# mhalushka/miRge3.0

Hardware: NVIDIA B200
Metric: M reads/s trim+collapse+annotate (higher is better)
Workload: dtype u8/int32

## Files before the change

### mirge3.0_b200/csrc/annotate.cu

```cuda
#include "common.cuh"

#include "annotate_verify.cuh"


__global__ void __launch_bounds__(256)
lib_kmers_kernel(mirge_library lib, uint32_t *__restrict__ kmer, uint8_t *__restrict__ valid) {
  const uint32_t p = blockIdx.x * 256u + threadIdx.x;
  if (p >= lib.n_bases) return;
  const uint32_t r = find_ref(lib, p);
  const uint32_t end = lib.d_ref_off[r + 1];
  uint32_t k = 0, v = 0;
  for (uint32_t i = 0; i < 16; ++i) {
    const uint32_t q = p + i;
    if (q >= end) break;
    if ((lib.d_nmask[q >> 5] >> (q & 31)) & 1u) break;
    k |= lib_base(lib.d_packed, q) << (2 * (15 - i));
    ++v;
  }
  kmer[p] = k;
  valid[p] = (uint8_t)v;
}

extern "C" int mirge_lib_kmers(mirge_ctx *ctx, const mirge_library *lib, uint32_t *d_kmer, uint8_t *d_valid, void *stream_) {
  if (!ctx) return MIRGE_ERR_ARG;
  if (!lib || !lib->d_packed || !lib->d_nmask || !lib->d_ref_off || !lib->d_ref_block || !d_kmer || !d_valid)
    MIRGE_FAIL(ctx, MIRGE_ERR_ARG, "lib_kmers: null buffer");
  if (lib->n_bases == 0 || lib->n_refs == 0) return MIRGE_OK;
  cudaStream_t stream = (cudaStream_t)stream_;
  MIRGE_CUDA(ctx, cudaSetDevice(ctx->device));
  lib_kmers_kernel<<<(lib->n_bases + 255) / 256, 256, 0, stream>>>(*lib, d_kmer, d_valid);
  MIRGE_LAUNCH_CHECK(ctx, "lib_kmers_kernel");
  return MIRGE_OK;
}

__global__ void __launch_bounds__(256)
lib_filter_kernel(const uint32_t *__restrict__ kmer, const uint8_t *__restrict__ valid, uint32_t n, uint32_t bases,
                  uint32_t *__restrict__ filter) {
  const uint32_t p = blockIdx.x * 256u + threadIdx.x;
  if (p >= n || valid[p] < bases) return;
  const uint32_t fi = bases >= 16 ? kmer[p] : (kmer[p] >> (32 - 2 * bases));
  atomicOr(filter + (fi >> 5), 1u << (fi & 31));
}

extern "C" int mirge_lib_filter(mirge_ctx *ctx, const uint32_t *d_kmer, const uint8_t *d_valid, uint32_t n_bases, uint32_t prefix_bases,
                                uint32_t *d_filter, void *stream_) {
  if (!ctx) return MIRGE_ERR_ARG;
  if (!d_kmer || !d_valid || !d_filter) MIRGE_FAIL(ctx, MIRGE_ERR_ARG, "lib_filter: null buffer");
  if (prefix_bases < 4 || prefix_bases > 16) MIRGE_FAIL(ctx, MIRGE_ERR_ARG, "lib_filter: prefix length must be 4..16");
  if (n_bases == 0) return MIRGE_OK;
  cudaStream_t stream = (cudaStream_t)stream_;
  MIRGE_CUDA(ctx, cudaSetDevice(ctx->device));
  MIRGE_CUDA(ctx, cudaMemsetAsync(d_filter, 0, (size_t)1 << (2 * prefix_bases - 3), stream));
  lib_filter_kernel<<<(n_bases + 255) / 256, 256, 0, stream>>>(d_kmer, d_valid, n_bases, prefix_bases, d_filter);
  MIRGE_LAUNCH_CHECK(ctx, "lib_filter_kernel");
  return MIRGE_OK;
}

__device__ __forceinline__ uint32_t mix32(uint32_t x) {
  x ^= x >> 16;
  x *= 0x7feb352du;
  x ^= x >> 15;
  x *= 0x846ca68bu;
  x ^= x >> 16;
  return x;
}
__device__ __forceinline__ bool filter16_pass(const mirge_library &lib, uint32_t kmer) {
  const uint32_t fi = mix32(kmer) >> (32 - lib.filter16_bits);
  return (lib.d_filter16[fi >> 5] >> (fi & 31)) & 1u;
}

__global__ void __launch_bounds__(256)
lib_filter16_kernel(const uint32_t *__restrict__ kmer, const uint8_t *__restrict__ valid, uint32_t n, uint32_t bits,
                    uint32_t *__restrict__ filter) {
  const uint32_t p = blockIdx.x * 256u + threadIdx.x;
  if (p >= n || valid[p] < 16) return;
  const uint32_t fi = mix32(kmer[p]) >> (32 - bits);
  atomicOr(filter + (fi >> 5), 1u << (fi & 31));
}

extern "C" int mirge_lib_filter16(mirge_ctx *ctx, const uint32_t *d_kmer, const uint8_t *d_valid, uint32_t n_bases, uint32_t bits,
                                  uint32_t *d_filter16, void *stream_) {
  if (!ctx) return MIRGE_ERR_ARG;
  if (!d_kmer || !d_valid || !d_filter16) MIRGE_FAIL(ctx, MIRGE_ERR_ARG, "lib_filter16: null buffer");
  if (bits < 16 || bits > 30) MIRGE_FAIL(ctx, MIRGE_ERR_ARG, "lib_filter16: 16..30 bits");
  cudaStream_t stream = (cudaStream_t)stream_;
  MIRGE_CUDA(ctx, cudaSetDevice(ctx->device));
  MIRGE_CUDA(ctx, cudaMemsetAsync(d_filter16, 0, (size_t)1 << (bits - 3), stream));
  if (n_bases == 0) return MIRGE_OK;
  lib_filter16_kernel<<<(n_bases + 255) / 256, 256, 0, stream>>>(d_kmer, d_valid, n_bases, bits, d_filter16);
  MIRGE_LAUNCH_CHECK(ctx, "lib_filter16_kernel");
  return MIRGE_OK;
}


#define MAX_PIECES 4
#define MAX_ROUNDS 10

struct RoundSet {
  int n;
  mirge_library lib[MAX_ROUNDS];
  mirge_round_policy pol[MAX_ROUNDS];
};

#define COOP_QW 6
struct WarpScratch {
  uint32_t qw[32][COOP_QW], qnx[32][COOP_QW];
  uint32_t lo[32][MAX_PIECES], hi[32][MAX_PIECES], off[32][MAX_PIECES];
  uint32_t len[32];
  uint32_t pref[33];
  unsigned long long best[32];
};

__device__ __forceinline__ uint64_t search_round(const mirge_library &lib, const mirge_round_policy &pol, bool active,
                                                 const uint32_t *qw, const uint32_t *qnx, int L, bool has_exc, WarpScratch &ws,
                                                 bool &republish, int lane) {
  uint32_t p_lo[MAX_PIECES], p_hi[MAX_PIECES], p_off[MAX_PIECES];
#pragma unroll
  for (int i = 0; i < MAX_PIECES; ++i) p_lo[i] = p_hi[i] = p_off[i] = 0;
  if (lib.max_ref_len && (uint32_t)L > lib.max_ref_len) active = false;
  const int R = pol.seed_len == 0 ? L : min(pol.seed_len, L);
  const int np = pol.seed_mm + 1;
  const bool degenerate = active && (R < MIN_SEED * np);
  const int nw = (L + 15) >> 4;
  if (active && !degenerate) {
    for (int pi = 0; pi < np; ++pi) {
      const int a = piece_bound(pi, R, np), b = piece_bound(pi + 1, R, np);
      const int s = min(16, b - a);
      if (has_exc && query_has_n(qnx, a, b)) continue;
      const uint32_t span = (s == 16) ? 0u : ((1u << (2 * (16 - s))) - 1u);
      const uint32_t k_lo = query_kmer16(qw, a, nw) & ~span, k_hi = k_lo | span;
      if (s == 16 && lib.filter16_bits && lib.filter_bases < 16) {
        if (!filter16_pass(lib, k_lo)) continue;
      } else if (lib.filter_bases && (uint32_t)s >= lib.filter_bases) {
        const uint32_t fi = lib.filter_bases >= 16 ? k_lo : (k_lo >> (32 - 2 * lib.filter_bases));
        if (!((lib.d_filter[fi >> 5] >> (fi & 31)) & 1u)) continue;
      }
      const uint32_t bsh = 32 - lib.bucket_bits;
      uint32_t l = lib.d_idx_bucket[k_lo >> bsh], h = lib.d_idx_bucket[(k_hi >> bsh) + 1];
      const uint32_t hi0 = h;
      while (l < h) { const uint32_t mid = (l + h) >> 1; if (lib.d_idx_kmer[mid] < k_lo) l = mid + 1; else h = mid; }
      p_lo[pi] = l;
      h = hi0;
      while (l < h) { const uint32_t mid = (l + h) >> 1; if (lib.d_idx_kmer[mid] <= k_hi) l = mid + 1; else h = mid; }
      p_hi[pi] = l;
      p_off[pi] = (uint32_t)a;
    }
  }
  uint64_t best = MIRGE_NO_HIT;
  uint32_t total = 0;
#pragma unroll
  for (int i = 0; i < MAX_PIECES; ++i) total += p_hi[i] - p_lo[i];
  const bool shared = active && !degenerate && total > 0 && nw <= COOP_QW;
  if (degenerate) {
    for (uint32_t r = 0; r < lib.n_refs; ++r) {
      const uint32_t lo = lib.d_ref_off[r], hi = lib.d_ref_off[r + 1];
      for (uint64_t a = lo; a + L <= hi; ++a) {
        const uint64_t h = verify(lib, qw, qnx, L, pol, R, a, (uint32_t)a);
        if (h < best) best = h;
      }
    }
  } else if (active && total > 0 && !shared) {
#pragma unroll
    for (int pi = 0; pi < MAX_PIECES; ++pi)
      for (uint32_t e = p_lo[pi]; e < p_hi[pi]; ++e) {
        const uint32_t pos = lib.d_idx_pos[e];
        if (pos < p_off[pi]) continue;
        const uint64_t h = verify(lib, qw, qnx, L, pol, R, pos - p_off[pi], pos);
        if (h < best) best = h;
      }
  }
  const unsigned sm = __ballot_sync(0xffffffffu, shared);
  if (sm == 0) return best;
  uint32_t incl = shared ? total : 0u;
#pragma unroll
  for (int d = 1; d < 32; d <<= 1) {
    const uint32_t x = __shfl_up_sync(0xffffffffu, incl, d);
    if (lane >= d) incl += x;
  }
  const uint32_t T = __shfl_sync(0xffffffffu, incl, 31);
  ws.pref[lane + 1] = incl;
  if (lane == 0) ws.pref[0] = 0;
  if (shared) {
    if (republish) {
      for (int w = 0; w < nw; ++w) { ws.qw[lane][w] = qw[w]; ws.qnx[lane][w] = qnx[w]; }
      republish = false;
    }
#pragma unroll
    for (int pi = 0; pi < MAX_PIECES; ++pi) { ws.lo[lane][pi] = p_lo[pi]; ws.hi[lane][pi] = p_hi[pi]; ws.off[lane][pi] = p_off[pi]; }
    ws.len[lane] = (uint32_t)L;
    ws.best[lane] = MIRGE_NO_HIT;
  }
  __syncwarp();
  for (uint32_t w = lane; w < T; w += 32) {
    int o = 0;
#pragma unroll
    for (int st = 16; st > 0; st >>= 1)
      if (ws.pref[o + st] <= w) o += st;
    uint32_t j = w - ws.pref[o];
    int pi = 0;
#pragma unroll
    for (int q = 0; q < MAX_PIECES - 1; ++q) {
      const uint32_t c = ws.hi[o][pi] - ws.lo[o][pi];
      if (j >= c && pi == q) { j -= c; ++pi; }
    }
    const uint32_t pos = lib.d_idx_pos[ws.lo[o][pi] + j], off = ws.off[o][pi];
    if (pos < off) continue;
    const int oL = (int)ws.len[o];
    const int oR = pol.seed_len == 0 ? oL : min(pol.seed_len, oL);
    const uint64_t h = verify(lib, ws.qw[o], ws.qnx[o], oL, pol, oR, pos - off, pos);
    if (h != MIRGE_NO_HIT) atomicMin(&ws.best[o], (unsigned long long)h);
  }
  __syncwarp();
  if (shared) {
    const uint64_t b = ws.best[lane];
    if (b < best) best = b;
  }
  return best;
}

__global__ void __launch_bounds__(ANN_THREADS, 10)
annotate_kernel(const __grid_constant__ RoundSet rs, mirge_table t, uint64_t n_keys, uint8_t *__restrict__ annot_round,
                uint64_t *__restrict__ hit) {
  __shared__ WarpScratch s_ws[ANN_THREADS / 32];
  const uint64_t slot = (uint64_t)blockIdx.x * ANN_THREADS + threadIdx.x;
  const int lane = threadIdx.x & 31, warp = threadIdx.x >> 5;
  const bool in_range = slot < n_keys;
  const uint64_t id = slot;
  uint32_t qw[QW_MAX], qnx[QW_MAX];
  KeyView kv;
  kv.pay = kv.exc = nullptr; kv.len = kv.nexc = 0;
  int cur_qs = -1, cur_qe = -1, tlen = -1;
  uint32_t state = 0xFF;
  if (in_range) {
    kv = key_view(t.d_arena + t.d_key_ref[id]);
    state = annot_round[id];
  }
  const int len = kv.len, nexc = kv.nexc;
  uint64_t my_hit = MIRGE_NO_HIT;
  int my_round = -1;
  bool republish = true;
  for (int ri = 0; ri < rs.n; ++ri) {
    const mirge_round_policy &pol = rs.pol[ri];
    bool active = in_range;
    if (active) {
      if (pol.select == MIRGE_SELECT_LEN_LT26) active = len < 26;
      else if (pol.select == MIRGE_SELECT_LEN_GT25) active = len > 25;
      else active = state == 0xFF;
    }
    int L = 0;
    if (active) {
      int qs, qe;
      active = round_window(kv, pol, tlen, qs, qe);
      if (active) {
        L = qe - qs;
        if (qs != cur_qs || qe != cur_qe) {
          build_query(kv, qs, qe, qw, qnx);
          cur_qs = qs;
          cur_qe = qe;
          republish = true;
        }
      }
    }
    const uint64_t best = search_round(rs.lib[ri], pol, active, qw, qnx, L, nexc > 0, s_ws[warp], republish, lane);
    if (active && best != MIRGE_NO_HIT) {
      state = (uint32_t)pol.round;
      my_round = pol.round;
      my_hit = best;
    }
  }
  if (my_round >= 0) {
    annot_round[id] = (uint8_t)my_round;
    hit[id] = my_hit;
  }
}

__global__ void __launch_bounds__(ANN_THREADS)
allhits_kernel(mirge_library lib, mirge_round_policy pol, mirge_table t, const uint32_t *__restrict__ ids, uint64_t n,
               const uint64_t *__restrict__ hit, int fill, uint32_t *__restrict__ counts, const uint64_t *__restrict__ offs,
               uint64_t *__restrict__ out) {
  const uint64_t i = (uint64_t)blockIdx.x * ANN_THREADS + threadIdx.x;
  if (i >= n) return;
  const uint32_t id = ids[i];
  const uint64_t want_mm = hit[id] >> 56;
  const KeyView kv = key_view(t.d_arena + t.d_key_ref[id]);
  uint32_t qw[QW_MAX], qnx[QW_MAX];
  int tlen = -1, qs, qe;
  uint32_t k = 0;
  const uint64_t o0 = fill ? offs[i] : 0;
  if (round_window(kv, pol, tlen, qs, qe)) {
    build_query(kv, qs, qe, qw, qnx);
    const int L = qe - qs, nw = (L + 15) >> 4;
    const int R = pol.seed_len == 0 ? L : min(pol.seed_len, L);
    const int np = pol.seed_mm + 1;
#define ALLHITS_TAKE(h_)                                    \
    if ((h_) != MIRGE_NO_HIT && ((h_) >> 56) == want_mm) {  \
      if (fill) out[o0 + k] = (h_);                         \
      ++k;                                                  \
    }
    if (R < MIN_SEED * np) {
      for (uint32_t r = 0; r < lib.n_refs; ++r) {
        const uint32_t lo = lib.d_ref_off[r], hi = lib.d_ref_off[r + 1];
        for (uint64_t a = lo; a + L <= hi; ++a) {
          const uint64_t h = verify(lib, qw, qnx, L, pol, R, a, (uint32_t)a);
          ALLHITS_TAKE(h)
        }
      }
    } else {
      for (int pi = 0; pi < np; ++pi) {
        const int a = piece_bound(pi, R, np), b = piece_bound(pi + 1, R, np);
        const int s = min(16, b - a);
        if (kv.nexc > 0 && query_has_n(qnx, a, b)) continue;
        const uint32_t span = (s == 16) ? 0u : ((1u << (2 * (16 - s))) - 1u);
        const uint32_t k_lo = query_kmer16(qw, a, nw) & ~span, k_hi = k_lo | span;
        const uint32_t bsh = 32 - lib.bucket_bits;
        uint32_t l = lib.d_idx_bucket[k_lo >> bsh], h = lib.d_idx_bucket[(k_hi >> bsh) + 1];
        const uint32_t hi0 = h;
        while (l < h) { const uint32_t mid = (l + h) >> 1; if (lib.d_idx_kmer[mid] < k_lo) l = mid + 1; else h = mid; }
        const uint32_t e0 = l;
        h = hi0;
        while (l < h) { const uint32_t mid = (l + h) >> 1; if (lib.d_idx_kmer[mid] <= k_hi) l = mid + 1; else h = mid; }
        for (uint32_t e = e0; e < l; ++e) {
          const uint32_t pos = lib.d_idx_pos[e];
          if (pos < (uint32_t)a) continue;
          const uint64_t hh = verify(lib, qw, qnx, L, pol, R, pos - (uint32_t)a, pos);
          ALLHITS_TAKE(hh)
        }
      }
    }
#undef ALLHITS_TAKE
  }
  if (!fill) counts[i] = k;
}


__device__ __forceinline__ uint32_t round_mask(const RoundSet &rs, const KeyView &kv, uint32_t state) {
  uint32_t qw[QW_MAX], qnx[QW_MAX];
  int cur_qs = -1, cur_qe = -1, tlen = -1;
  const int len = kv.len;
  const bool has_exc = kv.nexc > 0;
  uint32_t mask = 0;
  for (int ri = 0; ri < rs.n; ++ri) {
    const mirge_round_policy &pol = rs.pol[ri];
    const mirge_library &lib = rs.lib[ri];
    bool active;
    if (pol.select == MIRGE_SELECT_LEN_LT26) active = len < 26;
    else if (pol.select == MIRGE_SELECT_LEN_GT25) active = len > 25;
    else active = state == 0xFF;
    if (!active) continue;
    int qs, qe;
    if (!round_window(kv, pol, tlen, qs, qe)) continue;
    const int L = qe - qs;
    if (lib.max_ref_len && (uint32_t)L > lib.max_ref_len) continue;
    if (qs != cur_qs || qe != cur_qe) {
      build_query(kv, qs, qe, qw, qnx);
      cur_qs = qs;
      cur_qe = qe;
    }
    const int R = pol.seed_len == 0 ? L : min(pol.seed_len, L);
    const int np = pol.seed_mm + 1;
    const int nw = (L + 15) >> 4;
    bool pass = false;
    if (R < MIN_SEED * np) {
      pass = true;
    } else {
      for (int pi = 0; pi < np; ++pi) {
        const int a = piece_bound(pi, R, np), b = piece_bound(pi + 1, R, np);
        const int s = min(16, b - a);
        if (has_exc && query_has_n(qnx, a, b)) continue;
        if (s == 16 && lib.filter16_bits && lib.filter_bases < 16) {
          pass |= filter16_pass(lib, query_kmer16(qw, a, nw));
        } else if (lib.filter_bases && (uint32_t)s >= lib.filter_bases) {
          const uint32_t span = (s == 16) ? 0u : ((1u << (2 * (16 - s))) - 1u);
          const uint32_t k_lo = query_kmer16(qw, a, nw) & ~span;
          const uint32_t fi = lib.filter_bases >= 16 ? k_lo : (k_lo >> (32 - 2 * lib.filter_bases));
          pass |= ((lib.d_filter[fi >> 5] >> (fi & 31)) & 1u) != 0u;
        } else {
          pass = true;
        }
      }
    }
    if (pass) mask |= 1u << ri;
  }
  return mask;
}

#define LEAN_WORDS 8
#define MASK_THREADS 256
template <int S>
__device__ __forceinline__ uint32_t lean_word16(const uint32_t *col, int p) {
  const int wi = p >> 4, sh = 2 * (p & 15);
  return __funnelshift_r(col[wi * S], col[(wi + 1) * S], sh);
}
template <int S>
__device__ __forceinline__ uint32_t lean_kmer16(const uint32_t *col, int p) {
  const uint32_t v = lean_word16<S>(col, p);
  const uint32_t r = __brev(v);
  return ((r >> 1) & 0x55555555u) | ((r & 0x55555555u) << 1);
}

template <int S>
__device__ __forceinline__ bool lean_window(const uint32_t *col, int len, const mirge_round_policy &pol, int &tlen, int &qs, int &qe) {
  qs = 0;
  qe = len;
  if (pol.strip_polyT) {
    if (tlen < 0) {
      int tpos = len;
      while (tpos > 0 && ((col[((tpos - 1) >> 4) * S] >> (2 * ((tpos - 1) & 15))) & 3u) == 3u) --tpos;
      tlen = tpos;
    }
    if (len - tlen < 3) return false;
    qe = tlen;
  }
  qs += pol.trim5;
  qe -= pol.trim3;
  return qe > qs;
}

__device__ __forceinline__ uint32_t round_mask_lean(const RoundSet &rs, const uint32_t *col, int len, uint32_t state) {
  int tlen = -1;
  uint32_t mask = 0;
  for (int ri = 0; ri < rs.n; ++ri) {
    const mirge_round_policy &pol = rs.pol[ri];
    const mirge_library &lib = rs.lib[ri];
    bool active;
    if (pol.select == MIRGE_SELECT_LEN_LT26) active = len < 26;
    else if (pol.select == MIRGE_SELECT_LEN_GT25) active = len > 25;
    else active = state == 0xFF;
    if (!active) continue;
    int qs, qe;
    if (!lean_window<MASK_THREADS>(col, len, pol, tlen, qs, qe)) continue;
    const int L = qe - qs;
    if (lib.max_ref_len && (uint32_t)L > lib.max_ref_len) continue;
    const int R = pol.seed_len == 0 ? L : min(pol.seed_len, L);
    const int np = pol.seed_mm + 1;
    bool pass = false;
    if (R < MIN_SEED * np) {
      pass = true;
    } else {
      int a = 0;
      for (int pi = 0; pi < np; ++pi) {
        const int b = piece_bound(pi + 1, R, np);
        const int s = min(16, b - a);
        const uint32_t k16 = lean_kmer16<MASK_THREADS>(col, qs + a);
        if (s == 16 && lib.filter16_bits && lib.filter_bases < 16) {
          pass |= filter16_pass(lib, k16);
        } else if (lib.filter_bases && (uint32_t)s >= lib.filter_bases) {
          const uint32_t fi = lib.filter_bases >= 16 ? k16 : (k16 >> (32 - 2 * lib.filter_bases));
          pass |= ((lib.d_filter[fi >> 5] >> (fi & 31)) & 1u) != 0u;
        } else {
          pass = true;
        }
        a = b;
      }
    }
    if (pass) mask |= 1u << ri;
  }
  return mask;
}

__global__ void __launch_bounds__(MASK_THREADS)
annot_mask_kernel(const __grid_constant__ RoundSet rs, mirge_table t, uint64_t n_keys, const uint8_t *__restrict__ annot_round,
                  uint16_t *__restrict__ masks) {
  __shared__ uint32_t s_pay[LEAN_WORDS + 2][MASK_THREADS];
  const uint64_t id = (uint64_t)blockIdx.x * MASK_THREADS + threadIdx.x;
  if (id >= n_keys) return;
  const uint32_t *key = t.d_arena + t.d_key_ref[id];
  const uint32_t state = annot_round[id];
  const KeyView kv = key_view(key);
  const int npay = (kv.len + 15) >> 4;
  uint32_t mask;
  if (kv.nexc == 0 && npay <= LEAN_WORDS) {
    uint32_t *col = &s_pay[0][threadIdx.x];
#pragma unroll
    for (int w = 0; w < LEAN_WORDS + 2; ++w) col[w * MASK_THREADS] = w < npay ? kv.pay[w] : 0u;
    mask = round_mask_lean(rs, col, kv.len, state);
  } else {
    mask = round_mask(rs, kv, state);
  }
  masks[id] = (uint16_t)mask;
}

#ifndef LEAN_MAX_CAND
#define LEAN_MAX_CAND 12
#endif
template <int S>
__device__ __forceinline__ bool search_lean(const mirge_library &lib, const mirge_round_policy &pol, const uint32_t *col, int qs,
                                            int L, uint64_t &best) {
  if (lib.max_ref_len && (uint32_t)L > lib.max_ref_len) return true;
  const int R = pol.seed_len == 0 ? L : min(pol.seed_len, L);
  const int np = pol.seed_mm + 1;
  if (R < MIN_SEED * np) return false;
  uint32_t p_lo[MAX_PIECES], p_hi[MAX_PIECES];
  uint32_t total = 0;
  int a = 0;
#pragma unroll
  for (int pi = 0; pi < MAX_PIECES; ++pi) {
    p_lo[pi] = p_hi[pi] = 0;
    if (pi < np) {
      const int b = piece_bound(pi + 1, R, np);
      const int s = min(16, b - a);
      const uint32_t k16 = lean_kmer16<S>(col, qs + a);
      const uint32_t span = (s == 16) ? 0u : ((1u << (2 * (16 - s))) - 1u);
      const uint32_t k_lo = k16 & ~span, k_hi = k_lo | span;
      bool look = true;
      if (s == 16 && lib.filter16_bits && lib.filter_bases < 16) {
        look = filter16_pass(lib, k_lo);
      } else if (lib.filter_bases && (uint32_t)s >= lib.filter_bases) {
        const uint32_t fi = lib.filter_bases >= 16 ? k_lo : (k_lo >> (32 - 2 * lib.filter_bases));
        look = (lib.d_filter[fi >> 5] >> (fi & 31)) & 1u;
      }
      if (look) {
        const uint32_t bsh = 32 - lib.bucket_bits;
        uint32_t l = lib.d_idx_bucket[k_lo >> bsh], h = lib.d_idx_bucket[(k_hi >> bsh) + 1];
        const uint32_t hi0 = h;
        while (l < h) { const uint32_t mid = (l + h) >> 1; if (lib.d_idx_kmer[mid] < k_lo) l = mid + 1; else h = mid; }
        p_lo[pi] = l;
        h = hi0;
        while (l < h) { const uint32_t mid = (l + h) >> 1; if (lib.d_idx_kmer[mid] <= k_hi) l = mid + 1; else h = mid; }
        p_hi[pi] = l;
        total += p_hi[pi] - p_lo[pi];
      }
      a = b;
    }
  }
  if (total > LEAN_MAX_CAND) return false;
  const int nw = (L + 15) >> 4;
  a = 0;
#pragma unroll
  for (int pi = 0; pi < MAX_PIECES; ++pi) {
    if (pi < np) {
      for (uint32_t e = p_lo[pi]; e < p_hi[pi]; ++e) {
        const uint32_t pos = lib.d_idx_pos[e];
        if (pos < (uint32_t)a) continue;
        const uint64_t astart = pos - (uint32_t)a;
        int mm = 0, smm = 0;
        for (int w = 0; w < nw && mm >= 0; ++w) {
          uint32_t x = lean_word16<S>(col, qs + 16 * w) ^ lib_word16(lib.d_packed, astart + 16 * (uint64_t)w);
          x = (x | (x >> 1)) & 0x55555555u;
          const int rem = L - 16 * w;
          if (rem < 16) x &= (1u << (2 * rem)) - 1u;
          if (x) {
            mm += __popc(x);
            const int srem = R - 16 * w;
            if (srem >= 16) smm += __popc(x);
            else if (srem > 0) smm += __popc(x & ((1u << (2 * srem)) - 1u));
            if (mm > pol.total_mm || smm > pol.seed_mm) mm = -1;
          }
        }
        if (mm < 0) continue;
        const uint32_t r = find_ref(lib, pos);
        const uint32_t rlo = lib.d_ref_off[r], rhi = lib.d_ref_off[r + 1];
        if (astart < rlo || astart + (uint64_t)L > rhi) continue;
        if (ref_has_n(lib, astart, astart + L)) continue;
        const uint64_t hword = ((uint64_t)mm << 56) | ((uint64_t)r << 28) | (uint64_t)(astart - rlo);
        if (hword < best) best = hword;
      }
      a = piece_bound(pi + 1, R, np);
    }
  }
  return true;
}

#define SUB_KEYS 256
struct WarpTile {
  uint16_t mask[SUB_KEYS];
  uint16_t list[SUB_KEYS];
  uint8_t state[SUB_KEYS];
  uint32_t pay[LEAN_WORDS + 2][32];
};

struct GeneralList {
  unsigned long long *count;
  uint32_t *id;
  uint8_t *round;
};

__global__ void __launch_bounds__(ANN_THREADS, 10)
annot_search_kernel(const __grid_constant__ RoundSet rs, mirge_table t, uint64_t n_keys, const uint16_t *__restrict__ masks,
                    uint8_t *__restrict__ annot_round, uint64_t *__restrict__ hit, const GeneralList gl) {
  __shared__ WarpTile s_wt[ANN_THREADS / 32];
  const int lane = threadIdx.x & 31, warp = threadIdx.x >> 5;
  WarpTile &W = s_wt[warp];
  const uint64_t tile0 = ((uint64_t)blockIdx.x * (ANN_THREADS / 32) + warp) * SUB_KEYS;
  if (tile0 >= n_keys) return;
  const uint32_t n_tile = (uint32_t)min((uint64_t)SUB_KEYS, n_keys - tile0);
  uint32_t any = 0;
  for (uint32_t k = lane; k < SUB_KEYS; k += 32) {
    const uint32_t m = k < n_tile ? masks[tile0 + k] : 0u;
    W.mask[k] = (uint16_t)m;
    W.state[k] = k < n_tile ? annot_round[tile0 + k] : (uint8_t)0;
    any |= m;
  }
  any = __reduce_or_sync(0xffffffffu, any);
  __syncwarp();
  for (int ri = 0; ri < rs.n; ++ri) {
    if (!((any >> ri) & 1u)) continue;
    const mirge_round_policy &pol = rs.pol[ri];
    uint32_t cnt = 0;
    for (uint32_t k0 = 0; k0 < SUB_KEYS; k0 += 32) {
      const uint32_t k = k0 + lane;
      bool p = (W.mask[k] >> ri) & 1u;
      if (p && pol.select == MIRGE_SELECT_UNANNOTATED) p = W.state[k] == 0xFF;
      const unsigned bal = __ballot_sync(0xffffffffu, p);
      if (p) W.list[cnt + __popc(bal & ((1u << lane) - 1u))] = (uint16_t)k;
      cnt += __popc(bal);
    }
    __syncwarp();
    for (uint32_t base = 0; base < cnt; base += 32) {
      const uint32_t idx = base + lane;
      const bool active = idx < cnt;
      const uint32_t k = active ? W.list[idx] : 0u;
      const uint64_t id = tile0 + k;
      uint64_t best = MIRGE_NO_HIT;
      bool general = false;
      if (active) {
        const KeyView kv = key_view(t.d_arena + t.d_key_ref[id]);
        const int npay = (kv.len + 15) >> 4;
        general = true;
        if (kv.nexc == 0 && npay <= LEAN_WORDS) {
          uint32_t *col = &W.pay[0][lane];
#pragma unroll
          for (int w = 0; w < LEAN_WORDS + 2; ++w) col[w * 32] = w < npay ? kv.pay[w] : 0u;
          int qs, qe, tlen = -1;
          if (!lean_window<32>(col, kv.len, pol, tlen, qs, qe)) general = false;
          else general = !search_lean<32>(rs.lib[ri], pol, col, qs, qe - qs, best);
        }
      }
      const unsigned gm = __ballot_sync(0xffffffffu, general);
      if (gm) {
        const int leader = __ffs(gm) - 1;
        unsigned long long gb = 0;
        if (lane == leader) gb = atomicAdd(gl.count, (unsigned long long)__popc(gm));
        gb = __shfl_sync(0xffffffffu, gb, leader);
        if (general) {
          const unsigned long long e = gb + __popc(gm & ((1u << lane) - 1u));
          gl.id[e] = (uint32_t)id;
          gl.round[e] = (uint8_t)ri;
          W.mask[k] = 0;
        }
      }
      if (active && best != MIRGE_NO_HIT) {
        W.state[k] = (uint8_t)pol.round;
        annot_round[id] = (uint8_t)pol.round;
        hit[id] = best;
      }
    }
    __syncwarp();
  }
}

__global__ void __launch_bounds__(ANN_THREADS, 10)
annot_general_kernel(const __grid_constant__ RoundSet rs, mirge_table t, const GeneralList gl, uint8_t *__restrict__ annot_round,
                     uint64_t *__restrict__ hit) {
  __shared__ WarpScratch s_ws[ANN_THREADS / 32];
  const unsigned long long n = *gl.count;
  if ((uint64_t)blockIdx.x * ANN_THREADS >= n) return;
  const uint64_t i = (uint64_t)blockIdx.x * ANN_THREADS + threadIdx.x;
  const int lane = threadIdx.x & 31, warp = threadIdx.x >> 5;
  const bool in_range = i < n;
  const uint64_t id = in_range ? gl.id[i] : 0;
  const int first = in_range ? gl.round[i] : rs.n;
  uint32_t qw[QW_MAX], qnx[QW_MAX];
  KeyView kv;
  kv.pay = kv.exc = nullptr; kv.len = kv.nexc = 0;
  int cur_qs = -1, cur_qe = -1, tlen = -1;
  uint32_t state = 0xFF;
  if (in_range) {
    kv = key_view(t.d_arena + t.d_key_ref[id]);
    state = annot_round[id];
  }
  const int len = kv.len, nexc = kv.nexc;
  uint64_t my_hit = MIRGE_NO_HIT;
  int my_round = -1;
  bool republish = true;
  const int lo = __reduce_min_sync(0xffffffffu, first);
  for (int ri = lo; ri < rs.n; ++ri) {
    const mirge_round_policy &pol = rs.pol[ri];
    bool active = in_range && ri >= first;
    if (active) {
      if (pol.select == MIRGE_SELECT_LEN_LT26) active = len < 26;
      else if (pol.select == MIRGE_SELECT_LEN_GT25) active = len > 25;
      else active = state == 0xFF;
    }
    int L = 0;
    if (active) {
      int qs, qe;
      active = round_window(kv, pol, tlen, qs, qe);
      if (active) {
        L = qe - qs;
        if (qs != cur_qs || qe != cur_qe) {
          build_query(kv, qs, qe, qw, qnx);
          cur_qs = qs;
          cur_qe = qe;
          republish = true;
        }
      }
    }
    const uint64_t best = search_round(rs.lib[ri], pol, active, qw, qnx, L, nexc > 0, s_ws[warp], republish, lane);
    if (active && best != MIRGE_NO_HIT) {
      state = (uint32_t)pol.round;
      my_round = pol.round;
      my_hit = best;
    }
  }
  if (my_round >= 0) {
    annot_round[id] = (uint8_t)my_round;
    hit[id] = my_hit;
  }
}

extern "C" uint64_t mirge_annotate_scratch_bytes(uint64_t n_keys) {
  const uint64_t n = (n_keys + 7) & ~7ull;
  return 16 + 2 * n + 4 * n + n;
}

static int check_round(mirge_ctx *ctx, const mirge_library *lib, const mirge_round_policy *policy) {
  if (!lib->d_packed || !lib->d_nmask || !lib->d_ref_off || !lib->d_idx_kmer || !lib->d_idx_pos || !lib->d_idx_bucket ||
      !lib->d_ref_block)
    MIRGE_FAIL(ctx, MIRGE_ERR_ARG, "annotate: library has no index");
  if (lib->ref_block_shift > 20) MIRGE_FAIL(ctx, MIRGE_ERR_ARG, "annotate: ref_block_shift out of range");
  if (lib->filter_bases && (!lib->d_filter || lib->filter_bases < 4 || lib->filter_bases > 16))
    MIRGE_FAIL(ctx, MIRGE_ERR_ARG, "annotate: bad prefix filter");
  if (lib->filter16_bits && (!lib->d_filter16 || lib->filter16_bits < 16 || lib->filter16_bits > 30))
    MIRGE_FAIL(ctx, MIRGE_ERR_ARG, "annotate: bad 16-mer filter");
  if (lib->bucket_bits < 1 || lib->bucket_bits > 28) MIRGE_FAIL(ctx, MIRGE_ERR_ARG, "annotate: bucket_bits out of range");
  if (policy->seed_mm < 0 || policy->seed_mm > 3 || policy->total_mm < policy->seed_mm || policy->trim5 < 0 || policy->trim3 < 0)
    MIRGE_FAIL(ctx, MIRGE_ERR_ARG, "annotate: unsupported policy");
  if (lib->n_refs >= (1u << 28)) MIRGE_FAIL(ctx, MIRGE_ERR_ARG, "annotate: too many references");
  return MIRGE_OK;
}

extern "C" int mirge_annotate_rounds(mirge_ctx *ctx, const mirge_library *libs, const mirge_round_policy *policies, int n_rounds,
                                     const mirge_table *t, uint64_t n_keys, uint8_t *d_annot_round, uint64_t *d_hit,
                                     void *d_scratch, void *stream_) {
  if (!ctx) return MIRGE_ERR_ARG;
  if (!libs || !policies || !t || !d_annot_round || !d_hit) MIRGE_FAIL(ctx, MIRGE_ERR_ARG, "annotate: null argument");
  if (n_keys > 0xFFFFFFFFull) MIRGE_FAIL(ctx, MIRGE_ERR_ARG, "annotate: more than 2^32 sequences in one call");
  if (n_rounds < 0 || n_rounds > MAX_ROUNDS) MIRGE_FAIL(ctx, MIRGE_ERR_ARG, "annotate: at most %d rounds per call", MAX_ROUNDS);
  if (n_keys == 0 || n_rounds == 0) return MIRGE_OK;
  RoundSet rs;
  rs.n = 0;
  for (int i = 0; i < n_rounds; ++i) {
    if (libs[i].n_refs == 0 || libs[i].n_bases == 0) continue;
    int rc = check_round(ctx, &libs[i], &policies[i]);
    if (rc) return rc;
    rs.lib[rs.n] = libs[i];
    rs.pol[rs.n] = policies[i];
    ++rs.n;
  }
  if (rs.n == 0) return MIRGE_OK;
  cudaStream_t stream = (cudaStream_t)stream_;
  MIRGE_CUDA(ctx, cudaSetDevice(ctx->device));
  if (d_scratch) {
    if ((uintptr_t)d_scratch & 7) MIRGE_FAIL(ctx, MIRGE_ERR_ARG, "annotate: misaligned scratch");
    const uint64_t n8 = (n_keys + 7) & ~7ull;
    GeneralList gl;
    gl.count = (unsigned long long *)d_scratch;
    uint16_t *masks = (uint16_t *)((uint8_t *)d_scratch + 16);
    gl.id = (uint32_t *)((uint8_t *)d_scratch + 16 + 2 * n8);
    gl.round = (uint8_t *)d_scratch + 16 + 6 * n8;
    MIRGE_CUDA(ctx, cudaMemsetAsync(gl.count, 0, 16, stream));
    annot_mask_kernel<<<(unsigned)((n_keys + MASK_THREADS - 1) / MASK_THREADS), MASK_THREADS, 0, stream>>>(rs, *t, n_keys, d_annot_round, masks);
    MIRGE_LAUNCH_CHECK(ctx, "annot_mask_kernel");
    const uint64_t per_cta = (uint64_t)SUB_KEYS * (ANN_THREADS / 32);
    annot_search_kernel<<<(unsigned)((n_keys + per_cta - 1) / per_cta), ANN_THREADS, 0, stream>>>(rs, *t, n_keys, masks, d_annot_round, d_hit, gl);
    MIRGE_LAUNCH_CHECK(ctx, "annot_search_kernel");
    annot_general_kernel<<<(unsigned)((n_keys + ANN_THREADS - 1) / ANN_THREADS), ANN_THREADS, 0, stream>>>(rs, *t, gl, d_annot_round, d_hit);
    MIRGE_LAUNCH_CHECK(ctx, "annot_general_kernel");
    return MIRGE_OK;
  }
  annotate_kernel<<<(unsigned)((n_keys + ANN_THREADS - 1) / ANN_THREADS), ANN_THREADS, 0, stream>>>(rs, *t, n_keys, d_annot_round, d_hit);
  MIRGE_LAUNCH_CHECK(ctx, "annotate_kernel");
  return MIRGE_OK;
}

extern "C" int mirge_annotate_round(mirge_ctx *ctx, const mirge_library *lib, const mirge_round_policy *policy, const mirge_table *t,
                                    uint64_t n_keys, uint8_t *d_annot_round, uint64_t *d_hit, void *stream_) {
  if (!ctx) return MIRGE_ERR_ARG;
  if (!lib || !policy) MIRGE_FAIL(ctx, MIRGE_ERR_ARG, "annotate: null argument");
  return mirge_annotate_rounds(ctx, lib, policy, 1, t, n_keys, d_annot_round, d_hit, nullptr, stream_);
}

extern "C" int mirge_annotate_allhits(mirge_ctx *ctx, const mirge_library *lib, const mirge_round_policy *policy, const mirge_table *t,
                                      const uint32_t *d_ids, uint64_t n_ids, const uint64_t *d_hit, int fill, uint32_t *d_counts,
                                      const uint64_t *d_offs, uint64_t *d_out, void *stream_) {
  if (!ctx) return MIRGE_ERR_ARG;
  if (!lib || !policy || !t || !d_ids || !d_hit) MIRGE_FAIL(ctx, MIRGE_ERR_ARG, "allhits: null argument");
  if (fill ? (!d_offs || !d_out) : !d_counts) MIRGE_FAIL(ctx, MIRGE_ERR_ARG, "allhits: null output buffer");
  if (n_ids == 0) return MIRGE_OK;
  int rc = check_round(ctx, lib, policy);
  if (rc) return rc;
  cudaStream_t stream = (cudaStream_t)stream_;
  MIRGE_CUDA(ctx, cudaSetDevice(ctx->device));
  allhits_kernel<<<(unsigned)((n_ids + ANN_THREADS - 1) / ANN_THREADS), ANN_THREADS, 0, stream>>>(*lib, *policy, *t, d_ids, n_ids, d_hit,
                                                                                                   fill, d_counts, d_offs, d_out);
  MIRGE_LAUNCH_CHECK(ctx, "allhits_kernel");
  return MIRGE_OK;
}
```

Baseline: 1229.

## Spread high-candidate lean searches across the warp and persist the general kernel

Lean keys with more seed candidates than LEAN_MAX_CAND used to fall back to the slow general kernel. Now their candidate verifications are spread over all lanes of the warp, using a prefix sum and shared per-lane state, with an atomicMin into a shared best. The general kernel becomes a grid-stride loop, launched with a grid capped at resident-block capacity. The new shared struct enlarges per-block shared memory and adds warp syncs, which could lower occupancy of the search kernel.

```diff
diff --git a/mirge3.0_b200/csrc/annotate.cu b/mirge3.0_b200/csrc/annotate.cu
--- a/mirge3.0_b200/csrc/annotate.cu
+++ b/mirge3.0_b200/csrc/annotate.cu
@@ -480,36 +480,73 @@
   masks[id] = (uint16_t)mask;
 }
 
+__device__ __forceinline__ uint64_t lean_verify(const mirge_library &lib, const mirge_round_policy &pol, const uint32_t *col, int qs,
+                                                int L, int R, uint32_t pos, uint32_t a) {
+  if (pos < a) return MIRGE_NO_HIT;
+  const uint64_t astart = pos - a;
+  const int nw = (L + 15) >> 4;
+  int mm = 0, smm = 0;
+  for (int w = 0; w < nw; ++w) {
+    uint32_t x = lean_word16<32>(col, qs + 16 * w) ^ lib_word16(lib.d_packed, astart + 16 * (uint64_t)w);
+    x = (x | (x >> 1)) & 0x55555555u;
+    const int rem = L - 16 * w;
+    if (rem < 16) x &= (1u << (2 * rem)) - 1u;
+    if (x) {
+      mm += __popc(x);
+      const int srem = R - 16 * w;
+      if (srem >= 16) smm += __popc(x);
+      else if (srem > 0) smm += __popc(x & ((1u << (2 * srem)) - 1u));
+      if (mm > pol.total_mm || smm > pol.seed_mm) return MIRGE_NO_HIT;
+    }
+  }
+  const uint32_t r = find_ref(lib, pos);
+  const uint32_t rlo = lib.d_ref_off[r], rhi = lib.d_ref_off[r + 1];
+  if (astart < rlo || astart + (uint64_t)L > rhi) return MIRGE_NO_HIT;
+  if (ref_has_n(lib, astart, astart + L)) return MIRGE_NO_HIT;
+  return ((uint64_t)mm << 56) | ((uint64_t)r << 28) | (uint64_t)(astart - rlo);
+}
+
 #ifndef LEAN_MAX_CAND
 #define LEAN_MAX_CAND 12
 #endif
-template <int S>
-__device__ __forceinline__ bool search_lean(const mirge_library &lib, const mirge_round_policy &pol, const uint32_t *col, int qs,
-                                            int L, uint64_t &best) {
-  if (lib.max_ref_len && (uint32_t)L > lib.max_ref_len) return true;
+struct LeanShare {
+  uint32_t lo[MAX_PIECES][32], hi[MAX_PIECES][32];
+  uint32_t qs[32], len[32];
+  uint32_t pref[33];
+  unsigned long long best[32];
+};
+
+__device__ __forceinline__ bool search_lean(const mirge_library &lib, const mirge_round_policy &pol, uint32_t (*pay)[32],
+                                            LeanShare &sh, int lane, bool active, int len, uint64_t &best) {
+  const uint32_t *col = &pay[0][lane];
+  int qs = 0, qe = 0, tlen = -1;
+  bool look = active && lean_window<32>(col, len, pol, tlen, qs, qe);
+  const int L = qe - qs;
+  if (lib.max_ref_len && (uint32_t)L > lib.max_ref_len) look = false;
   const int R = pol.seed_len == 0 ? L : min(pol.seed_len, L);
   const int np = pol.seed_mm + 1;
-  if (R < MIN_SEED * np) return false;
+  const bool degenerate = look && R < MIN_SEED * np;
+  if (degenerate) look = false;
   uint32_t p_lo[MAX_PIECES], p_hi[MAX_PIECES];
   uint32_t total = 0;
   int a = 0;
 #pragma unroll
   for (int pi = 0; pi < MAX_PIECES; ++pi) {
     p_lo[pi] = p_hi[pi] = 0;
-    if (pi < np) {
+    if (look && pi < np) {
       const int b = piece_bound(pi + 1, R, np);
       const int s = min(16, b - a);
-      const uint32_t k16 = lean_kmer16<S>(col, qs + a);
+      const uint32_t k16 = lean_kmer16<32>(col, qs + a);
       const uint32_t span = (s == 16) ? 0u : ((1u << (2 * (16 - s))) - 1u);
       const uint32_t k_lo = k16 & ~span, k_hi = k_lo | span;
-      bool look = true;
+      bool present = true;
       if (s == 16 && lib.filter16_bits && lib.filter_bases < 16) {
-        look = filter16_pass(lib, k_lo);
+        present = filter16_pass(lib, k_lo);
       } else if (lib.filter_bases && (uint32_t)s >= lib.filter_bases) {
         const uint32_t fi = lib.filter_bases >= 16 ? k_lo : (k_lo >> (32 - 2 * lib.filter_bases));
-        look = (lib.d_filter[fi >> 5] >> (fi & 31)) & 1u;
-      }
-      if (look) {
+        present = (lib.d_filter[fi >> 5] >> (fi & 31)) & 1u;
+      }
+      if (present) {
         const uint32_t bsh = 32 - lib.bucket_bits;
         uint32_t l = lib.d_idx_bucket[k_lo >> bsh], h = lib.d_idx_bucket[(k_hi >> bsh) + 1];
         const uint32_t hi0 = h;
@@ -523,42 +560,63 @@
       a = b;
     }
   }
-  if (total > LEAN_MAX_CAND) return false;
-  const int nw = (L + 15) >> 4;
-  a = 0;
-#pragma unroll
-  for (int pi = 0; pi < MAX_PIECES; ++pi) {
-    if (pi < np) {
-      for (uint32_t e = p_lo[pi]; e < p_hi[pi]; ++e) {
-        const uint32_t pos = lib.d_idx_pos[e];
-        if (pos < (uint32_t)a) continue;
-        const uint64_t astart = pos - (uint32_t)a;
-        int mm = 0, smm = 0;
-        for (int w = 0; w < nw && mm >= 0; ++w) {
-          uint32_t x = lean_word16<S>(col, qs + 16 * w) ^ lib_word16(lib.d_packed, astart + 16 * (uint64_t)w);
-          x = (x | (x >> 1)) & 0x55555555u;
-          const int rem = L - 16 * w;
-          if (rem < 16) x &= (1u << (2 * rem)) - 1u;
-          if (x) {
-            mm += __popc(x);
-            const int srem = R - 16 * w;
-            if (srem >= 16) smm += __popc(x);
-            else if (srem > 0) smm += __popc(x & ((1u << (2 * srem)) - 1u));
-            if (mm > pol.total_mm || smm > pol.seed_mm) mm = -1;
-          }
+  const bool share = total > LEAN_MAX_CAND;
+  if (!share && total > 0) {
+    a = 0;
+#pragma unroll
+    for (int pi = 0; pi < MAX_PIECES; ++pi) {
+      if (pi < np) {
+        for (uint32_t x = p_lo[pi]; x < p_hi[pi]; ++x) {
+          const uint64_t h = lean_verify(lib, pol, col, qs, L, R, lib.d_idx_pos[x], (uint32_t)a);
+          if (h < best) best = h;
         }
-        if (mm < 0) continue;
-        const uint32_t r = find_ref(lib, pos);
-        const uint32_t rlo = lib.d_ref_off[r], rhi = lib.d_ref_off[r + 1];
-        if (astart < rlo || astart + (uint64_t)L > rhi) continue;
-        if (ref_has_n(lib, astart, astart + L)) continue;
-        const uint64_t hword = ((uint64_t)mm << 56) | ((uint64_t)r << 28) | (uint64_t)(astart - rlo);
-        if (hword < best) best = hword;
-      }
-      a = piece_bound(pi + 1, R, np);
-    }
-  }
-  return true;
+        a = piece_bound(pi + 1, R, np);
+      }
+    }
+  }
+  if (__ballot_sync(0xffffffffu, share)) {
+    uint32_t incl = share ? total : 0u;
+#pragma unroll
+    for (int d = 1; d < 32; d <<= 1) {
+      const uint32_t x = __shfl_up_sync(0xffffffffu, incl, d);
+      if (lane >= d) incl += x;
+    }
+    const uint32_t T = __shfl_sync(0xffffffffu, incl, 31);
+    sh.pref[lane + 1] = incl;
+    if (lane == 0) sh.pref[0] = 0;
+    if (share) {
+#pragma unroll
+      for (int pi = 0; pi < MAX_PIECES; ++pi) { sh.lo[pi][lane] = p_lo[pi]; sh.hi[pi][lane] = p_hi[pi]; }
+      sh.qs[lane] = (uint32_t)qs;
+      sh.len[lane] = (uint32_t)L;
+      sh.best[lane] = MIRGE_NO_HIT;
+    }
+    __syncwarp();
+    for (uint32_t w = lane; w < T; w += 32) {
+      int o = 0;
+#pragma unroll
+      for (int st = 16; st > 0; st >>= 1)
+        if (sh.pref[o + st] <= w) o += st;
+      uint32_t j = w - sh.pref[o];
+      int pi = 0;
+#pragma unroll
+      for (int q = 0; q < MAX_PIECES - 1; ++q) {
+        const uint32_t c = sh.hi[pi][o] - sh.lo[pi][o];
+        if (j >= c && pi == q) { j -= c; ++pi; }
+      }
+      const int oL = (int)sh.len[o];
+      const int oR = pol.seed_len == 0 ? oL : min(pol.seed_len, oL);
+      const uint64_t h = lean_verify(lib, pol, &pay[0][o], (int)sh.qs[o], oL, oR, lib.d_idx_pos[sh.lo[pi][o] + j],
+                                     (uint32_t)piece_bound(pi, oR, np));
+      if (h != MIRGE_NO_HIT) atomicMin(&sh.best[o], (unsigned long long)h);
+    }
+    __syncwarp();
+    if (share) {
+      const uint64_t b = sh.best[lane];
+      if (b < best) best = b;
+    }
+  }
+  return !degenerate;
 }
 
 #define SUB_KEYS 256
@@ -567,6 +625,7 @@
   uint16_t list[SUB_KEYS];
   uint8_t state[SUB_KEYS];
   uint32_t pay[LEAN_WORDS + 2][32];
+  LeanShare share;
 };
 
 struct GeneralList {
@@ -612,20 +671,21 @@
       const uint32_t k = active ? W.list[idx] : 0u;
       const uint64_t id = tile0 + k;
       uint64_t best = MIRGE_NO_HIT;
-      bool general = false;
+      bool lean = false;
+      int len = 0;
       if (active) {
         const KeyView kv = key_view(t.d_arena + t.d_key_ref[id]);
         const int npay = (kv.len + 15) >> 4;
-        general = true;
-        if (kv.nexc == 0 && npay <= LEAN_WORDS) {
+        lean = kv.nexc == 0 && npay <= LEAN_WORDS;
+        len = kv.len;
+        if (lean) {
           uint32_t *col = &W.pay[0][lane];
 #pragma unroll
           for (int w = 0; w < LEAN_WORDS + 2; ++w) col[w * 32] = w < npay ? kv.pay[w] : 0u;
-          int qs, qe, tlen = -1;
-          if (!lean_window<32>(col, kv.len, pol, tlen, qs, qe)) general = false;
-          else general = !search_lean<32>(rs.lib[ri], pol, col, qs, qe - qs, best);
         }
       }
+      const bool searched = search_lean(rs.lib[ri], pol, W.pay, W.share, lane, active && lean, len, best);
+      const bool general = active && (!lean || !searched);
       const unsigned gm = __ballot_sync(0xffffffffu, general);
       if (gm) {
         const int leader = __ffs(gm) - 1;
@@ -644,6 +704,7 @@
         annot_round[id] = (uint8_t)pol.round;
         hit[id] = best;
       }
+      __syncwarp();
     }
     __syncwarp();
   }
@@ -654,58 +715,60 @@
                      uint64_t *__restrict__ hit) {
   __shared__ WarpScratch s_ws[ANN_THREADS / 32];
   const unsigned long long n = *gl.count;
-  if ((uint64_t)blockIdx.x * ANN_THREADS >= n) return;
-  const uint64_t i = (uint64_t)blockIdx.x * ANN_THREADS + threadIdx.x;
   const int lane = threadIdx.x & 31, warp = threadIdx.x >> 5;
-  const bool in_range = i < n;
-  const uint64_t id = in_range ? gl.id[i] : 0;
-  const int first = in_range ? gl.round[i] : rs.n;
-  uint32_t qw[QW_MAX], qnx[QW_MAX];
-  KeyView kv;
-  kv.pay = kv.exc = nullptr; kv.len = kv.nexc = 0;
-  int cur_qs = -1, cur_qe = -1, tlen = -1;
-  uint32_t state = 0xFF;
-  if (in_range) {
-    kv = key_view(t.d_arena + t.d_key_ref[id]);
-    state = annot_round[id];
-  }
-  const int len = kv.len, nexc = kv.nexc;
-  uint64_t my_hit = MIRGE_NO_HIT;
-  int my_round = -1;
-  bool republish = true;
-  const int lo = __reduce_min_sync(0xffffffffu, first);
-  for (int ri = lo; ri < rs.n; ++ri) {
-    const mirge_round_policy &pol = rs.pol[ri];
-    bool active = in_range && ri >= first;
-    if (active) {
-      if (pol.select == MIRGE_SELECT_LEN_LT26) active = len < 26;
-      else if (pol.select == MIRGE_SELECT_LEN_GT25) active = len > 25;
-      else active = state == 0xFF;
-    }
-    int L = 0;
-    if (active) {
-      int qs, qe;
-      active = round_window(kv, pol, tlen, qs, qe);
+  for (uint64_t base = (uint64_t)blockIdx.x * ANN_THREADS; base < n; base += (uint64_t)gridDim.x * ANN_THREADS) {
+    const uint64_t i = base + threadIdx.x;
+    const bool in_range = i < n;
+    const uint64_t id = in_range ? gl.id[i] : 0;
+    const int first = in_range ? gl.round[i] : rs.n;
+    uint32_t qw[QW_MAX], qnx[QW_MAX];
+    KeyView kv;
+    kv.pay = kv.exc = nullptr; kv.len = kv.nexc = 0;
+    int cur_qs = -1, cur_qe = -1, tlen = -1;
+    uint32_t state = 0xFF;
+    if (in_range) {
+      kv = key_view(t.d_arena + t.d_key_ref[id]);
+      state = annot_round[id];
+    }
+    const int len = kv.len, nexc = kv.nexc;
+    uint64_t my_hit = MIRGE_NO_HIT;
+    int my_round = -1;
+    bool republish = true;
+    const int lo = __reduce_min_sync(0xffffffffu, first);
+    for (int ri = lo; ri < rs.n; ++ri) {
+      const mirge_round_policy &pol = rs.pol[ri];
+      bool active = in_range && ri >= first;
       if (active) {
-        L = qe - qs;
-        if (qs != cur_qs || qe != cur_qe) {
-          build_query(kv, qs, qe, qw, qnx);
-          cur_qs = qs;
-          cur_qe = qe;
-          republish = true;
+        if (pol.select == MIRGE_SELECT_LEN_LT26) active = len < 26;
+        else if (pol.select == MIRGE_SELECT_LEN_GT25) active = len > 25;
+        else active = state == 0xFF;
+      }
+      int L = 0;
+      if (active) {
+        int qs, qe;
+        active = round_window(kv, pol, tlen, qs, qe);
+        if (active) {
+          L = qe - qs;
+          if (qs != cur_qs || qe != cur_qe) {
+            build_query(kv, qs, qe, qw, qnx);
+            cur_qs = qs;
+            cur_qe = qe;
+            republish = true;
+          }
         }
       }
-    }
-    const uint64_t best = search_round(rs.lib[ri], pol, active, qw, qnx, L, nexc > 0, s_ws[warp], republish, lane);
-    if (active && best != MIRGE_NO_HIT) {
-      state = (uint32_t)pol.round;
-      my_round = pol.round;
-      my_hit = best;
-    }
-  }
-  if (my_round >= 0) {
-    annot_round[id] = (uint8_t)my_round;
-    hit[id] = my_hit;
+      const uint64_t best = search_round(rs.lib[ri], pol, active, qw, qnx, L, nexc > 0, s_ws[warp], republish, lane);
+      if (active && best != MIRGE_NO_HIT) {
+        state = (uint32_t)pol.round;
+        my_round = pol.round;
+        my_hit = best;
+      }
+    }
+    if (my_round >= 0) {
+      annot_round[id] = (uint8_t)my_round;
+      hit[id] = my_hit;
+    }
+    __syncwarp();
   }
 }
 
@@ -765,7 +828,11 @@
     const uint64_t per_cta = (uint64_t)SUB_KEYS * (ANN_THREADS / 32);
     annot_search_kernel<<<(unsigned)((n_keys + per_cta - 1) / per_cta), ANN_THREADS, 0, stream>>>(rs, *t, n_keys, masks, d_annot_round, d_hit, gl);
     MIRGE_LAUNCH_CHECK(ctx, "annot_search_kernel");
-    annot_general_kernel<<<(unsigned)((n_keys + ANN_THREADS - 1) / ANN_THREADS), ANN_THREADS, 0, stream>>>(rs, *t, gl, d_annot_round, d_hit);
+    int sms = 0, per_sm = 0;
+    MIRGE_CUDA(ctx, cudaDeviceGetAttribute(&sms, cudaDevAttrMultiProcessorCount, ctx->device));
+    MIRGE_CUDA(ctx, cudaOccupancyMaxActiveBlocksPerMultiprocessor(&per_sm, annot_general_kernel, ANN_THREADS, 0));
+    const uint64_t g_cap = (n_keys + ANN_THREADS - 1) / ANN_THREADS, g_res = (uint64_t)sms * (per_sm > 0 ? per_sm : 1);
+    annot_general_kernel<<<(unsigned)(g_cap < g_res ? g_cap : g_res), ANN_THREADS, 0, stream>>>(rs, *t, gl, d_annot_round, d_hit);
     MIRGE_LAUNCH_CHECK(ctx, "annot_general_kernel");
     return MIRGE_OK;
   }
diff --git a/profiles/annot_work.py b/profiles/annot_work.py
--- /dev/null
+++ b/profiles/annot_work.py
@@ -0,0 +1,143 @@
+import argparse
+import ctypes as C
+import os
+import statistics
+import subprocess
+import sys
+
+sys.dont_write_bytecode = True
+
+
+def main():
+    ap = argparse.ArgumentParser()
+    ap.add_argument("--config", type=int, default=2)
+    ap.add_argument("--root", default=os.path.dirname(os.path.dirname(os.path.abspath(__file__))))
+    ap.add_argument("--reps", type=int, default=5)
+    ap.add_argument("--label", default="")
+    a = ap.parse_args()
+    sys.path.insert(0, os.path.abspath(a.root))
+    import numpy as np
+    import torch
+
+    import bench
+    import mirge_b200
+    from mirge_b200 import abi
+    from mirge_b200 import device as D
+    from mirge_b200 import libraries as LB
+    from mirge_b200 import manifoldAlign as MA
+    from mirge_b200 import synth
+
+    argv, sys.argv = sys.argv, ["bench.py", "--config", str(a.config)]
+    args = bench.parse_args()
+    sys.argv = argv
+    smi = subprocess.run(["nvidia-smi", "--query-gpu=name,power.limit,clocks.max.sm", "--format=csv,noheader"],
+                         capture_output=True, text=True).stdout.strip().splitlines()
+    print("tree: %s %s" % (os.path.abspath(a.root), a.label))
+    print("gpu: %s" % (smi[0] if smi else "unknown"))
+    print("workload: %s" % args.workload)
+
+    dev = D.Device(0)
+    torch.cuda.set_device(dev.tdev)
+    libs = synth.make_libraries(mrna_count=args.mrna)
+    lset = LB.LibrarySet.from_fasta_dict(dev, libs.fasta_dict())
+    eng = D.DigestEngine(dev, synth.trim_config_for(args.config, args.count_mode))
+    fq = bench.sample_fastq(libs, args.config, 0, args.reads, False, dev.tdev)
+    table = D.CollapseTable(dev, min_keys=1 << 22)
+    eng.digest_device(fq, table, args.batch_mb << 20)
+    table.drain()
+    del fq
+    keys = MA.KeySet.from_table(table)
+    n = keys.n
+    n_rounds = 10 if args.spike else 9
+    pols = LB.round_policies()[:n_rounds]
+    lib_arr = (abi.Library * n_rounds)(*[lset[LB.ROUND_LIBS[r]].struct for r in range(n_rounds)])
+    pol_arr = (abi.RoundPolicy * n_rounds)(*pols)
+    nbytes = dev.lib.mirge_annotate_scratch_bytes(n)
+    scratch = torch.empty(nbytes // 8 + 1, dtype=torch.int64, device=dev.tdev)
+    annot = torch.empty(n, dtype=torch.uint8, device=dev.tdev)
+    hit = torch.empty(n, dtype=torch.int64, device=dev.tdev)
+
+    def run():
+        annot.fill_(0xFF)
+        hit.fill_(-1)
+        dev.check(dev.lib.mirge_annotate_rounds(dev.ctx, lib_arr, pol_arr, n_rounds, C.byref(keys.struct), n, MA._ptr(annot),
+                                                MA._ptr(hit), MA._ptr(scratch), dev.stream()))
+
+    run()
+    torch.cuda.synchronize()
+    print("unique sequences: %d   scratch: %.2f GB (%.1f bytes per sequence)" % (n, nbytes / 1e9, nbytes / max(n, 1)))
+
+    ref = keys.key_ref[:n].long() & 0xFFFFFFFF
+    hdr = keys.arena[ref].long() & 0xFFFFFFFF
+    klen = (hdr & 0xFFFF).cpu().numpy()
+    nexc = (hdr >> 16).cpu().numpy()
+    ar = annot.cpu().numpy()
+    raw = scratch.view(torch.uint8)
+    n8 = (n + 7) & ~7
+    if nbytes == 16 + 7 * n8:
+        gcount = int(raw[:8].view(torch.int64).item())
+        masks = raw[16:16 + 2 * n].view(torch.int16).cpu().numpy().astype(np.int64) & 0xFFFF
+        gid = raw[16 + 2 * n8:16 + 2 * n8 + 4 * gcount].view(torch.int32).cpu().numpy().astype(np.int64) & 0xFFFFFFFF
+        grnd = raw[16 + 6 * n8:16 + 6 * n8 + gcount].cpu().numpy()
+        lists = None
+    else:
+        base = (16 - scratch.data_ptr() % 16) % 16
+        ctr = raw[base:base + 256].view(torch.int32).cpu().numpy().astype(np.int64)
+        lists, gcount = ctr[:n_rounds], int(ctr[21])
+        o = base + 256 + 52 * n8
+        gid = raw[o:o + 4 * gcount].view(torch.int32).cpu().numpy().astype(np.int64) & 0xFFFFFFFF
+        grnd = raw[o + 4 * n8:o + 4 * n8 + gcount].cpu().numpy()
+        masks = None
+    print("\nround  annotated  " + ("mask_bit_set  searched" if masks is not None else "list_size"))
+    for r in range(n_rounds):
+        ann = int((ar == r).sum())
+        if masks is not None:
+            bit = (masks >> r) & 1 == 1
+            searched = bit if pols[r].select != abi.SELECT_UNANNOTATED else bit & ((ar >= r) | (ar == 0xFF))
+            print("%5d  %9d  %12d  %8d" % (r, ann, int(bit.sum()), int(searched.sum())))
+        else:
+            print("%5d  %9d  %9d" % (r, ann, int(lists[r])))
+    print("unannotated: %d" % int((ar == 0xFF).sum()))
+    lean = (nexc == 0) & (klen <= 128)
+    if masks is not None:
+        print("sequences with a non-zero mask: %d (lean %d)" % (int((masks != 0).sum()), int(((masks != 0) & lean).sum())))
+    print("\ngeneral pass list: %d" % gcount)
+    reasons = np.where(nexc[gid] > 0, 0, np.where(klen[gid] > 128, 1, 2))
+    names = ["exception words", "over 128 bases", "lean key"]
+    for r in range(n_rounds):
+        sel = grnd == r
+        if sel.any():
+            print("  entered at round %d: %8d  " % (r, int(sel.sum())) +
+                  "  ".join("%s %d" % (names[k], int((reasons[sel] == k).sum())) for k in range(3)))
+
+    ev = []
+    for _ in range(a.reps):
+        s, e = torch.cuda.Event(enable_timing=True), torch.cuda.Event(enable_timing=True)
+        s.record()
+        run()
+        e.record()
+        torch.cuda.synchronize()
+        ev.append(s.elapsed_time(e))
+    print("\nannotation call (CUDA events, includes the two result fills): median %.3f ms, min %.3f, max %.3f over %d"
+          % (statistics.median(ev), min(ev), max(ev), a.reps))
+
+    from torch.profiler import ProfilerActivity, profile
+
+    with profile(activities=[ProfilerActivity.CUDA]) as prof:
+        for _ in range(a.reps):
+            run()
+        torch.cuda.synchronize()
+    rows = []
+    for evt in prof.key_averages():
+        t = getattr(evt, "device_time_total", None)
+        if t is None:
+            t = getattr(evt, "cuda_time_total", 0.0)
+        if t > 0:
+            rows.append((t / a.reps / 1000.0, evt.count // a.reps, evt.key))
+    print("\nper-kernel time per call (torch.profiler, %d calls)" % a.reps)
+    for ms, cnt, key in sorted(rows, reverse=True):
+        print("  %8.3f ms  %3d launches  %s" % (ms, cnt, key[:90]))
+
+
+if __name__ == "__main__":
+    main()
```

New measurement: 1213, median of 6. 0.987x the previous value.
